# PREDICT-EPFL/piqp

Hardware: AMD Instinct MI355X
Metric: KKT factor+solve/sec (per IPM iter) (higher is better)
Workload: dtype f64; 1 GPU; dense QP n=4096 p=0 m_ineq=4096 (BASELINE configs[1]), kkt_solver=dense_cholesky, 1 update_scalings_and_factor + 2 KKTSystem::solve per step, inputs resident in HBM; n=4096, p=0, m=4096, parallelism=independent QP replicas x1

## Files before the change

piqp_amd/csrc/dense_kernels.hip:

```cpp
#include "dense_kernels.hpp"

#include <algorithm>
#include <map>
#include <mutex>
#include <stdexcept>
#include <utility>
#include <vector>
#include <cstdlib>
#include <cstdio>
#include <cstring>

namespace pq {
namespace dense {

typedef double d4 __attribute__((ext_vector_type(4)));
typedef double d2 __attribute__((ext_vector_type(2)));

__device__ __forceinline__ double readlane_d(double v, int srclane)
{
    long long bits = __double_as_longlong(v);
    int lo = (int)(bits & 0xffffffffll), hi = (int)(bits >> 32);
    lo = __builtin_amdgcn_readlane(lo, srclane);
    hi = __builtin_amdgcn_readlane(hi, srclane);
    return __longlong_as_double(((long long)hi << 32) | (unsigned int)lo);
}

template <bool FROM_LOWER>
__global__ __launch_bounds__(256) void k_symmetrize_upper(const double* __restrict__ Pu, int ldu, int n, double* __restrict__ Pf, double* __restrict__ pdiag)
{
    __shared__ double tile[32][33];
    const int r0 = blockIdx.x * 32, c0 = blockIdx.y * 32;
    const bool lower_tile = r0 > c0;
    const int sr0 = lower_tile ? c0 : r0, sc0 = lower_tile ? r0 : c0;
    const int tx = threadIdx.x & 31, ty = threadIdx.x >> 5;
    for (int cc = ty; cc < 32; cc += 8) {
        if constexpr (FROM_LOWER) {
            int c = sc0 + tx, r = sr0 + cc;
            tile[tx][cc] = (r < n && c < n) ? Pu[c + (size_t)r * ldu] : 0.0;
        } else {
            int r = sr0 + tx, c = sc0 + cc;
            tile[cc][tx] = (r < n && c < n) ? Pu[r + (size_t)c * ldu] : 0.0;
        }
    }
    __syncthreads();
    for (int cc = ty; cc < 32; cc += 8) {
        int i = r0 + tx, j = c0 + cc;
        if (i < n && j < n) {
            double v;
            if (lower_tile) v = tile[tx][cc];
            else if (r0 == c0) v = (tx <= cc) ? tile[cc][tx] : tile[tx][cc];
            else v = tile[cc][tx];
            Pf[i + (size_t)j * n] = v;
            if (i == j && pdiag) pdiag[i] = v;
        }
    }
}

#ifndef PQ_FUSE_TS
#define PQ_FUSE_TS 0
#endif
constexpr bool AGENT_OPERANDS = false;
constexpr bool FUSE_TS_ON = PQ_FUSE_TS != 0;
constexpr int TS = 128;
constexpr int BK = 16;
constexpr int LDS_LD = TS + 16;
constexpr int SYRK_LDS_BYTES = 2 * 2 * BK * LDS_LD * (int)sizeof(double);

__device__ __forceinline__ double ld_agent(const double* p);
__device__ __forceinline__ void st_agent(double* p, double v);
typedef __attribute__((address_space(1))) int gint;
__device__ __forceinline__ int ldi_agent(const int* p) { return __hip_atomic_load((const gint*)p, __ATOMIC_RELAXED, __HIP_MEMORY_SCOPE_AGENT); }
__device__ __forceinline__ void sti_agent(int* p, int v) { __hip_atomic_store((gint*)p, v, __ATOMIC_RELAXED, __HIP_MEMORY_SCOPE_AGENT); }
__device__ __forceinline__ int addi_agent(int* p, int v) { return __hip_atomic_fetch_add((gint*)p, v, __ATOMIC_RELAXED, __HIP_MEMORY_SCOPE_AGENT); }
template <bool CHECK, int NT>
__device__ __forceinline__ void load_tile(const double* __restrict__ M, int ld, int r0, int k0, int nrows, int kdim, int tid, d2 (&v)[1024 / NT])
{
    const int r = r0 + 2 * (tid & 63);
#pragma unroll
    for (int it = 0; it < 1024 / NT; ++it) {
        const int k = k0 + it * (NT / 64) + (tid >> 6);
        const __attribute__((address_space(1))) double* Mg = (const __attribute__((address_space(1))) double*)M;
        if (!CHECK) {
            v[it] = *reinterpret_cast<const __attribute__((address_space(1))) d2*>(Mg + r + (size_t)k * ld);
        } else {
            d2 t = {0.0, 0.0};
// ... 217 lines not shown
#pragma unroll
                    for (int q = 0; q < GRP; ++q) {
                        const int kt = g0 + q;
                        if (kt < nkt) {
                            const double* Asb = A4 + q * BK * LDS_LD + wr * SUBR + (lane & 15);
                            const double* Bsb = B4 + q * BK * LDS_LD + wc * SUBC + (lane & 15);
#pragma unroll
                            for (int ks = 0; ks < 4; ++ks) {
                                const int kk = ks * 4 + (lane >> 4);
                                double af[MTR], bf[MTC];
#pragma unroll
                                for (int u = 0; u < MTR; ++u) af[u] = Asb[kk * LDS_LD + u * 16];
#pragma unroll
                                for (int u = 0; u < MTC; ++u) bf[u] = Bsb[kk * LDS_LD + u * 16];
#pragma unroll
                                for (int x = 0; x < MTC; ++x)
#pragma unroll
                                    for (int y = 0; y < MTR; ++y)
                                        acc[x][y] = __builtin_amdgcn_mfma_f64_16x16x4f64(bf[x], af[y], acc[x][y], 0, 0, 0);
                            }
                        }
                    }
                }
            }
        }
        __syncthreads();
    }
    if (dbg_tile) a.fuse_ts[86] = clock64();
    if (tr_tile) a.fuse_tr2[42] = wall_clock64();
    if (tr_row) a.fuse_tr2[51] = wall_clock64();
    if constexpr (!QUARTER) {
        if (a.fuse_cnt && tj == 0 && a.fuse_pack) return panel_follow<NT, MTC, MTR, PERSIST, ROWS / 16>(a, smem, acc, row0, wr, wc, ti == 1);
    }
    if (skip_wave) return true;
#pragma unroll
    for (int x = 0; x < MTC; ++x) {
#pragma unroll
        for (int y = 0; y < MTR; ++y) {
            const int gi = row0 + wr * SUBR + y * 16 + (lane & 15);
#pragma unroll
            for (int r = 0; r < 4; ++r) {
                const int gj = col0 + wc * SUBC + x * 16 + (lane >> 4) + 4 * r;
                if (gi < a.n && gj < a.n && gi >= gj && gj < a.ncol) {
                    double* cp = a.C + (size_t)gi + (size_t)gj * a.ldc;
                    if (PERSIST) st_agent(cp, acc[x][y][r]);
                    else if constexpr (SUMSUB) *(__attribute__((address_space(1))) double*)cp = cfetch[x][y][r] - acc[x][y][r];
                    else *cp = acc[x][y][r];
                }
            }
        }
    }
    if (dbg_tile) { asm volatile("s_waitcnt vmcnt(0)" ::: "memory"); a.fuse_ts[87] = clock64(); }
    if (tr_tile) { a.fuse_tr2[43] = wall_clock64(); asm volatile("s_waitcnt vmcnt(0)" ::: "memory"); a.fuse_tr2[44] = wall_clock64(); }
    return true;
}

template <int EPI, int WR, int WC>
__device__ __forceinline__ void syrk_lower_body(const SyrkArgs& a, const int block_x)
{
    constexpr int NT = 64 * WR * WC;
    constexpr int MTR = 8 / WR, MTC = 8 / WC;
    constexpr int SUBR = TS / WR, SUBC = TS / WC;
    extern __shared__ __attribute__((aligned(16))) double smem[];
    double* As = smem;
    double* Bs = smem + 2 * BK * LDS_LD;

    int bid = block_x;
    if constexpr (EPI == EPI_SUBTRACT_POTRF) {
        if (bid < FUSE_ROLES) { fused_next_diag<NT, false>(a, smem, bid); return; }
        bid -= FUSE_ROLES - 1;
        const int T = (a.n + TS - 1) / TS;
        int ti, tj;
        if (bid <= T - 1) { ti = bid; tj = 0; }
        else {
            const int bb = bid - T;
            int t2 = (int)((sqrt(8.0 * (double)bb + 1.0) - 1.0) * 0.5);
            while ((t2 + 1) * (t2 + 2) / 2 <= bb) ++t2;
            while (t2 * (t2 + 1) / 2 > bb) --t2;
            ti = t2 + 1; tj = bb - t2 * (t2 + 1) / 2 + 1;
        }
        (void)fused_tile<NT, false>(a, ti, tj, smem);
        return;
    } else {
    const int b = a.tile_begin + bid / a.k_split;
    const int kslice = bid % a.k_split;
    int ti, tj;
    if (a.tile_order) {
        const int pk = a.tile_order[b];
        ti = pk >> 16; tj = pk & 0xffff;
    } else {
        ti = (int)((sqrt(8.0 * (double)b + 1.0) - 1.0) * 0.5);
        while ((ti + 1) * (ti + 2) / 2 <= b) ++ti;
        while (ti * (ti + 1) / 2 > b) --ti;
        tj = b - ti * (ti + 1) / 2;
    }
    const int row0 = ti * TS, col0 = tj * TS;
    if (col0 >= a.ncol) return;

    const int tid = threadIdx.x, lane = tid & 63, wave = tid >> 6;
    const int wr = wave / WC, wc = wave % WC;
    const bool edge = (row0 + TS > a.n) || (col0 + TS > a.n) || a.unaligned;
    const bool skip_wave = (ti == tj) && ((wr + 1) * SUBR <= wc * SUBC);

    d4 acc[MTC][MTR];
#pragma unroll
    for (int x = 0; x < MTC; ++x)
#pragma unroll
        for (int y = 0; y < MTR; ++y) acc[x][y] = (d4){0.0, 0.0, 0.0, 0.0};

    const int nkt_all = (a.kdim + BK - 1) / BK;
    const int kt_per = (nkt_all + a.k_split - 1) / a.k_split;
    const int kt_begin = kslice * kt_per;
    const int nkt = max(0, min(nkt_all, kt_begin + kt_per) - kt_begin);
    d2 va[1024 / NT], vb[1024 / NT];
    if (nkt > 0) {
        const int k0 = kt_begin * BK;
        const bool chk = edge || (k0 + BK > a.kdim);
        if (chk) { load_tile<true, NT>(a.A, a.lda, row0, k0, a.n, a.kdim, tid, va); load_tile<true, NT>(a.B, a.ldb, col0, k0, a.n, a.kdim, tid, vb); scale_tile<true, NT>(a.w, k0, a.kdim, tid, vb); }
        else { load_tile<false, NT>(a.A, a.lda, row0, k0, a.n, a.kdim, tid, va); load_tile<false, NT>(a.B, a.ldb, col0, k0, a.n, a.kdim, tid, vb); scale_tile<false, NT>(a.w, k0, a.kdim, tid, vb); }
        store_tile<NT>(As, tid, va);
        store_tile<NT>(Bs, tid, vb);
    }
    __syncthreads();

    for (int kt = 0; kt < nkt; ++kt) {
        const int cur = kt & 1;
        const bool more = (kt + 1 < nkt);
        if (more) {
            const int k0 = (kt_begin + kt + 1) * BK;
            const bool chk = edge || (k0 + BK > a.kdim);
            if (chk) { load_tile<true, NT>(a.A, a.lda, row0, k0, a.n, a.kdim, tid, va); load_tile<true, NT>(a.B, a.ldb, col0, k0, a.n, a.kdim, tid, vb); scale_tile<true, NT>(a.w, k0, a.kdim, tid, vb); }
            else { load_tile<false, NT>(a.A, a.lda, row0, k0, a.n, a.kdim, tid, va); load_tile<false, NT>(a.B, a.ldb, col0, k0, a.n, a.kdim, tid, vb); scale_tile<false, NT>(a.w, k0, a.kdim, tid, vb); }
        }
        if (!skip_wave) {
            const double* Asb = As + cur * BK * LDS_LD + wr * SUBR + (lane & 15);
            const double* Bsb = Bs + cur * BK * LDS_LD + wc * SUBC + (lane & 15);
#pragma unroll
            for (int ks = 0; ks < 4; ++ks) {
                const int kk = ks * 4 + (lane >> 4);
                double af[MTR], bf[MTC];
#pragma unroll
                for (int q = 0; q < MTR; ++q) af[q] = Asb[kk * LDS_LD + q * 16];
#pragma unroll
                for (int q = 0; q < MTC; ++q) bf[q] = Bsb[kk * LDS_LD + q * 16];
#pragma unroll
                for (int x = 0; x < MTC; ++x)
#pragma unroll
                    for (int y = 0; y < MTR; ++y)
                        acc[x][y] = __builtin_amdgcn_mfma_f64_16x16x4f64(bf[x], af[y], acc[x][y], 0, 0, 0);
            }
        }
        if (more) {
            store_tile<NT>(As + (cur ^ 1) * BK * LDS_LD, tid, va);
            store_tile<NT>(Bs + (cur ^ 1) * BK * LDS_LD, tid, vb);
        }
        __syncthreads();
    }

    if (skip_wave) return;
    if (a.part) {
        double* P = a.part + (size_t)block_x * TS * TS;
#pragma unroll
        for (int x = 0; x < MTC; ++x)
#pragma unroll
            for (int y = 0; y < MTR; ++y)
#pragma unroll
                for (int r = 0; r < 4; ++r)
                    P[(wr * SUBR + y * 16 + (lane & 15)) + (size_t)(wc * SUBC + x * 16 + (lane >> 4) + 4 * r) * TS] = acc[x][y][r];
        return;
    }
#pragma unroll
    for (int x = 0; x < MTC; ++x) {
#pragma unroll
        for (int y = 0; y < MTR; ++y) {
            const int gi = row0 + wr * SUBR + y * 16 + (lane & 15);
#pragma unroll
            for (int r = 0; r < 4; ++r) {
                const int gj = col0 + wc * SUBC + x * 16 + (lane >> 4) + 4 * r;
                if (gi < a.n && gj < a.n && gi >= gj && gj < a.ncol) {
                    const size_t ci = (size_t)gi + (size_t)gj * a.ldc;
                    const double v = acc[x][y][r];
                    if (EPI == EPI_ASSEMBLE) {
                        double base = a.Pfull[(size_t)gi + (size_t)gj * a.ldp];
                        if (gi == gj) base += a.x_reg[gi];
                        if (a.ATA) base += a.dinv * a.ATA[(size_t)gi + (size_t)gj * a.ldata];
                        ((__attribute__((address_space(1))) double*)a.C)[ci] = base + v;
                    } else if (EPI == EPI_SUBTRACT) {
                        ((__attribute__((address_space(1))) double*)a.C)[ci] -= v;
                    } else {
                        ((__attribute__((address_space(1))) double*)a.C)[ci] = v;
                    }
                }
            }
        }
    }
    }
}

template <int EPI, int WR, int WC>
__global__ __launch_bounds__(64 * WR * WC, (WR * WC == 4) ? 2 : (WR * WC == 8 ? 2 : 4)) void k_syrk_lower(SyrkArgs a)
{
    syrk_lower_body<EPI, WR, WC>(a, (int)blockIdx.x);
}

__device__ __forceinline__ bool front_panel(const FrontJob& j, int panel, int& k, int& nb, int& rs)
{
    k = panel * FACTOR_NB;
    if (k >= j.w) return false;
    nb = min(FACTOR_NB, j.w - k);
    rs = j.f - k - nb;
    return true;
}
template <int WR, int WC>
__global__ __launch_bounds__(64 * WR * WC, (WR * WC == 4) ? 2 : (WR * WC == 8 ? 2 : 4)) void k_syrk_lower_fronts(const FrontJob* __restrict__ jobs, int panel, int kind)
{
    const FrontJob j = jobs[blockIdx.y];
    if (kind >= 0 && j.kind != kind) return;
    int k, nb, rs;
    if (!front_panel(j, panel, k, nb, rs) || rs <= 0) return;
    const int T = (rs + TS - 1) / TS;
    if ((int)blockIdx.x >= T * (T + 1) / 2) return;
    SyrkArgs a;
    a.n = rs; a.kdim = nb;
    a.A = j.F + (k + nb) + (size_t)k * j.f; a.lda = j.f; a.B = a.A; a.ldb = j.f; a.w = j.dvec + k;
    a.C = j.F + (k + nb) + (size_t)(k + nb) * j.f; a.ldc = j.f;
    a.unaligned = ((j.f & 1) || (reinterpret_cast<uintptr_t>(a.A) & 15)) ? 1 : 0;
    if (j.multi) {
        a.ncol = j.w - (k + nb);
        if (a.ncol <= 0) return;
    }
    syrk_lower_body<EPI_SUBTRACT, WR, WC>(a, (int)blockIdx.x);
}
template <int WR, int WC>
__global__ __launch_bounds__(64 * WR * WC, (WR * WC == 4) ? 2 : (WR * WC == 8 ? 2 : 4)) void k_syrk_multi_fronts(const FrontJob* __restrict__ jobs)
{
    const FrontJob j = jobs[blockIdx.y];
    if (!j.multi || j.kind != 0) return;
    const int u = j.f - j.w;
    const int T = (u + TS - 1) / TS;
    if (u <= 0 || (int)blockIdx.x >= T * (T + 1) / 2) return;
    for (int k = 0; k < j.w; k += FACTOR_NB) {
        SyrkArgs a;
        a.n = u; a.kdim = min(FACTOR_NB, j.w - k);
        a.A = j.F + j.w + (size_t)k * j.f; a.lda = j.f; a.B = a.A; a.ldb = j.f; a.w = j.dvec + k;
        a.C = j.F + j.w + (size_t)j.w * j.f; a.ldc = j.f;
        a.unaligned = ((j.f & 1) || (reinterpret_cast<uintptr_t>(a.A) & 15)) ? 1 : 0;
        syrk_lower_body<EPI_SUBTRACT, WR, WC>(a, (int)blockIdx.x);
        __threadfence_block();
        __syncthreads();
    }
}

template <int SPLIT>
__global__ __launch_bounds__(512) void k_syrk_half_fronts(const FrontJob* __restrict__ jobs, int panel, int kind)
{
    const FrontJob j = jobs[blockIdx.y];
    if (kind >= 0 && j.kind != kind) return;
    int k, nb, rs;
    if (!front_panel(j, panel, k, nb, rs) || rs <= 0) return;
    const int T = (rs + TS - 1) / TS;
    const int b = (int)blockIdx.x / SPLIT, h = (int)blockIdx.x % SPLIT;
    if (b >= T * (T + 1) / 2) return;
    int ti = (int)((sqrt(8.0 * (double)b + 1.0) - 1.0) * 0.5);
    while ((ti + 1) * (ti + 2) / 2 <= b) ++ti;
    while (ti * (ti + 1) / 2 > b) --ti;
    const int tj = b - ti * (ti + 1) / 2;
    if (ti * TS + (TS / SPLIT) * h >= rs) return;
    SyrkArgs a;
    a.n = rs; a.kdim = nb;
    a.A = j.F + (k + nb) + (size_t)k * j.f; a.lda = j.f; a.B = a.A; a.ldb = j.f; a.w = j.dvec + k;
    a.C = j.F + (k + nb) + (size_t)(k + nb) * j.f; a.ldc = j.f;
    a.unaligned = ((j.f & 1) || (reinterpret_cast<uintptr_t>(a.A) & 15)) ? 1 : 0;
    if (j.multi) {
        a.ncol = j.w - (k + nb);
        if (a.ncol <= 0 || tj * TS >= a.ncol) return;
    }
    extern __shared__ __attribute__((aligned(16))) double smem[];
    (void)fused_tile<512, false, true, true, SPLIT == 4>(a, ti, tj, smem, h);
}

template <int EPI>
__global__ __launch_bounds__(256) void k_syrk_tail_reduce(SyrkArgs a)
{
    const int b = a.tile_begin + (int)blockIdx.x;
    int ti, tj;
    if (a.tile_order) {
        const int pk = a.tile_order[b];
        ti = pk >> 16; tj = pk & 0xffff;
    } else {
        ti = (int)((sqrt(8.0 * (double)b + 1.0) - 1.0) * 0.5);
        while ((ti + 1) * (ti + 2) / 2 <= b) ++ti;
        while (ti * (ti + 1) / 2 > b) --ti;
        tj = b - ti * (ti + 1) / 2;
    }
    const int row0 = ti * TS, col0 = tj * TS;
    const double* P0 = a.part + (size_t)blockIdx.x * a.k_split * TS * TS;
    {
        const int idx = (int)blockIdx.y * 256 + (int)threadIdx.x;
        const int li = idx & (TS - 1), lj = idx >> 7;
        const int gi = row0 + li, gj = col0 + lj;
        if (gi >= a.n || gj >= a.n || gi < gj) return;
        double v = 0.0;
#pragma unroll 8
        for (int sl = 0; sl < a.k_split; ++sl) v += P0[(size_t)sl * TS * TS + idx];
        const size_t ci = (size_t)gi + (size_t)gj * a.ldc;
        if (EPI == EPI_ASSEMBLE) {
            double base = a.Pfull[(size_t)gi + (size_t)gj * a.ldp];
            if (gi == gj) base += a.x_reg[gi];
            if (a.ATA) base += a.dinv * a.ATA[(size_t)gi + (size_t)gj * a.ldata];
            a.C[ci] = base + v;
        } else if (EPI == EPI_SUBTRACT) {
            a.C[ci] -= v;
        } else {
            a.C[ci] = v;
        }
    }
}

static int g_slots = 0;
static int syrk_slots()
{
    if (g_slots == 0) {
        int dev = 0, cus = 256;
        if (hipGetDevice(&dev) == hipSuccess) (void)hipDeviceGetAttribute(&cus, hipDeviceAttributeMultiprocessorCount, dev);
        g_slots = 2 * (cus > 0 ? cus : 256);
    }
    return g_slots;
}
static void syrk_tail_plan(int n, int kdim, int& rem, int& ksplit)
{
    const int T = div_up(n, TS);
    const int ntiles = T * (T + 1) / 2;
    const int slots = syrk_slots();
    const int nkt = div_up(kdim, BK);
    rem = ntiles % slots;
    ksplit = 1;
    if (ntiles > slots && rem > 0 && rem * 10 < slots * 6) {
        int s = slots / rem;
        s = std::min(s, nkt / 4);
        if (s >= 2) ksplit = s;
    }
    if (ksplit == 1) rem = 0;
}
size_t syrk_split_workspace_doubles(int n, int kdim)
{
    int rem, ks;
    syrk_tail_plan(n, kdim, rem, ks);
    return (size_t)rem * ks * TS * TS;
}

static const int* syrk_tile_order(int T)
{
    static std::mutex mu;
    static std::map<std::pair<int, int>, int*> cache;
    if (T < 16) return nullptr;
    int dev = 0;
    if (hipGetDevice(&dev) != hipSuccess) return nullptr;
    std::lock_guard<std::mutex> lk(mu);
    auto it = cache.find({dev, T});
    if (it != cache.end()) return it->second;
    constexpr int S = 8, NX = 8;
    std::vector<int> blocked;
    for (int SI = 0; SI * S < T; ++SI)
        for (int SJ = 0; SJ <= SI; ++SJ)
            for (int ti = SI * S; ti < std::min(T, SI * S + S); ++ti)
                for (int tj = SJ * S; tj < SJ * S + S && tj <= ti; ++tj) blocked.push_back(ti << 16 | tj);
    const int nt = (int)blocked.size();
    std::vector<int> start(NX + 1, 0);
    for (int x = 0; x < NX; ++x) start[x + 1] = start[x] + nt / NX + (x < nt % NX ? 1 : 0);
    std::vector<int> order(nt);
    for (int b = 0; b < nt; ++b) order[b] = blocked[start[b % NX] + b / NX];
    int* d = nullptr;
    if (hipMalloc(&d, sizeof(int) * nt) != hipSuccess) { (void)hipGetLastError(); cache[{dev, T}] = nullptr; return nullptr; }
    ++alloc_counter();
    if (hipMemcpy(d, order.data(), sizeof(int) * nt, hipMemcpyHostToDevice) != hipSuccess) { (void)hipGetLastError(); (void)hipFree(d); d = nullptr; }
    cache[{dev, T}] = d;
    return d;
}

void syrk_prepare(int n) { (void)syrk_tile_order(div_up(n, TS)); }

template <int EPI>
static void launch_syrk_t(SyrkArgs a, hipStream_t s, double* ws, size_t ws_doubles)
{
    const int T = div_up(a.n, TS);
    const int ntiles = T * (T + 1) / 2;
    int rem = 0, ks = 1;
    if (ws) syrk_tail_plan(a.n, a.kdim, rem, ks);
    if (rem > 0 && (size_t)rem * ks * TS * TS > ws_doubles) { rem = 0; ks = 1; }
    const int main_tiles = ntiles - rem;
    a.tile_begin = 0; a.k_split = 1; a.part = nullptr;
    const bool low_latency = a.kdim <= 256;
    a.tile_order = !low_latency ? syrk_tile_order(T) : nullptr;
    if (low_latency) hipLaunchKernelGGL((k_syrk_lower<EPI, 4, 4>), dim3(main_tiles), dim3(1024), SYRK_LDS_BYTES, s, a);
    else hipLaunchKernelGGL((k_syrk_lower<EPI, 2, 2>), dim3(main_tiles), dim3(256), SYRK_LDS_BYTES, s, a);
    if (rem > 0) {
        a.tile_begin = main_tiles; a.k_split = ks; a.part = ws;
        hipLaunchKernelGGL((k_syrk_lower<EPI, 2, 2>), dim3(rem * ks), dim3(256), SYRK_LDS_BYTES, s, a);
        hipLaunchKernelGGL(k_syrk_tail_reduce<EPI>, dim3(rem, TS * TS / 256), dim3(256), 0, s, a);
    }
}

void launch_syrk(int epi, const SyrkArgs& args_in, hipStream_t s, double* split_ws, size_t split_ws_doubles)
{
    SyrkArgs a = args_in;
    if (a.n <= 0) return;
    a.unaligned = ((a.lda & 1) || (a.ldb & 1) || (reinterpret_cast<uintptr_t>(a.A) & 15) || (reinterpret_cast<uintptr_t>(a.B) & 15)) ? 1 : 0;
    static PerDeviceOnce attr_set;
    attr_set([&] {
        PQ_HIP(hipFuncSetAttribute(reinterpret_cast<const void*>(k_syrk_lower<EPI_ASSEMBLE, 2, 2>), hipFuncAttributeMaxDynamicSharedMemorySize, SYRK_LDS_BYTES));
        PQ_HIP(hipFuncSetAttribute(reinterpret_cast<const void*>(k_syrk_lower<EPI_SUBTRACT, 2, 2>), hipFuncAttributeMaxDynamicSharedMemorySize, SYRK_LDS_BYTES));
        PQ_HIP(hipFuncSetAttribute(reinterpret_cast<const void*>(k_syrk_lower<EPI_STORE, 2, 2>), hipFuncAttributeMaxDynamicSharedMemorySize, SYRK_LDS_BYTES));
        PQ_HIP(hipFuncSetAttribute(reinterpret_cast<const void*>(k_syrk_lower<EPI_ASSEMBLE, 4, 4>), hipFuncAttributeMaxDynamicSharedMemorySize, SYRK_LDS_BYTES));
        PQ_HIP(hipFuncSetAttribute(reinterpret_cast<const void*>(k_syrk_lower<EPI_SUBTRACT, 4, 4>), hipFuncAttributeMaxDynamicSharedMemorySize, SYRK_LDS_BYTES));
        PQ_HIP(hipFuncSetAttribute(reinterpret_cast<const void*>(k_syrk_lower<EPI_STORE, 4, 4>), hipFuncAttributeMaxDynamicSharedMemorySize, SYRK_LDS_BYTES));
    });
    if (epi == EPI_SUBTRACT_POTRF) {
        static PerDeviceOnce fused_attr;
        fused_attr([&] {
            PQ_HIP(hipFuncSetAttribute(reinterpret_cast<const void*>(k_syrk_lower<EPI_SUBTRACT_POTRF, 4, 2>), hipFuncAttributeMaxDynamicSharedMemorySize, FUSED_LDS_BYTES));
        });
        const int T = div_up(a.n, TS);
        a.tile_begin = 0; a.k_split = 1; a.part = nullptr;
        if (!a.fuse_scratch || !a.fuse_flags || a.fuse_nb <= 0 || a.kdim > TS) throw std::runtime_error("fused trailing update: scratch / flags / panel width");
        hipLaunchKernelGGL((k_syrk_lower<EPI_SUBTRACT_POTRF, 4, 2>), dim3(T * (T + 1) / 2 + FUSE_ROLES - 1), dim3(512), FUSED_LDS_BYTES, s, a);
        PQ_HIP(hipGetLastError());
        return;
    }
    switch (epi) {
    case EPI_ASSEMBLE: launch_syrk_t<EPI_ASSEMBLE>(a, s, split_ws, split_ws_doubles); break;
    case EPI_SUBTRACT: launch_syrk_t<EPI_SUBTRACT>(a, s, split_ws, split_ws_doubles); break;
    default: launch_syrk_t<EPI_STORE>(a, s, split_ws, split_ws_doubles); break;
    }
    PQ_HIP(hipGetLastError());
}

__global__ __launch_bounds__(256) void k_assemble_no_g(int n, const double* __restrict__ Pf, const double* __restrict__ x_reg, const double* __restrict__ ATA, double dinv, double* __restrict__ C)
{
    const int j = blockIdx.y;
    const int i = blockIdx.x * 256 + threadIdx.x;
    if (i < n && i >= j) {
        double v = Pf[i + (size_t)j * n];
        if (i == j) v += x_reg[i];
        if (ATA) v += dinv * ATA[i + (size_t)j * n];
        C[i + (size_t)j * n] = v;
    }
}
void launch_assemble_no_g(int n, const double* Pf, const double* x_reg, const double* ATA, double dinv, double* C, hipStream_t s)
{
    if (n <= 0) return;
    hipLaunchKernelGGL(k_assemble_no_g, dim3(div_up(n, 256), n), dim3(256), 0, s, n, Pf, x_reg, ATA, dinv, C);
    PQ_HIP(hipGetLastError());
}


template <int NBLK, int LD, int NT = 256, bool TRANSPOSE = false>
__device__ __forceinline__ void stage_lower_block(const double* __restrict__ A, int lda, int nr, double* __restrict__ Ls, int tid)
{
    constexpr int PER_THREAD = NBLK * NBLK / NT;
    constexpr int BATCH = 16;
#pragma unroll 1
    for (int b0 = 0; b0 < PER_THREAD; b0 += BATCH) {
        double v[BATCH];
#pragma unroll
        for (int u = 0; u < BATCH; ++u) {
            const int idx = (b0 + u) * NT + tid;
            const int r = idx % NBLK, c = idx / NBLK;
            const bool ok = (r < nr) && (c < nr) && (r >= c);
            const double* p = ok ? (A + r + (size_t)c * lda) : A;
            const double t = *p;
            v[u] = ok ? t : ((r == c) ? 1.0 : 0.0);
        }
#pragma unroll
        for (int u = 0; u < BATCH; ++u) {
            const int idx = (b0 + u) * NT + tid;
            if (TRANSPOSE) Ls[(idx % NBLK) * LD + (idx / NBLK)] = v[u];
            else Ls[(idx / NBLK) * LD + (idx % NBLK)] = v[u];
        }
    }
}

__device__ __forceinline__ int tb_index(int bi, int bj) { return bi * (bi + 1) / 2 + bj; }
constexpr int TB_BLOCKS = 36;
constexpr int TB_DOUBLES = TB_BLOCKS * 256;
constexpr int POTRF_LDS_BYTES = (TB_DOUBLES + 8 * 32) * (int)sizeof(double);

__device__ __forceinline__ d4 tile_load(const double* __restrict__ blk, int lane)
{
    const double* p = blk + (lane >> 4) * 16 + (lane & 15);
    return (d4){p[0], p[64], p[128], p[192]};
}
__device__ __forceinline__ void tile_store(double* __restrict__ blk, int lane, d4 t)
{
    double* p = blk + (lane >> 4) * 16 + (lane & 15);
    p[0] = t[0]; p[64] = t[1]; p[128] = t[2]; p[192] = t[3];
}

__device__ __forceinline__ void wave_lds_sync()
{
    __builtin_amdgcn_fence(__ATOMIC_RELEASE, "wavefront");
    __builtin_amdgcn_wave_barrier();
    __builtin_amdgcn_fence(__ATOMIC_ACQUIRE, "wavefront");
}

constexpr int PIVOT_NEWTON = 2;
__device__ __forceinline__ double rsqrt_newton(double d)
// ... 2555 lines not shown
```

piqp_amd/csrc/dense_kernels.hpp:

```cpp
#pragma once

#include "common.hpp"

namespace pq {
namespace dense {

enum { EPI_ASSEMBLE = 0, EPI_SUBTRACT = 1, EPI_STORE = 2, EPI_SUBTRACT_POTRF = 3 };

struct SyrkArgs {
    int n = 0;
    int kdim = 0;
    const double* A = nullptr; int lda = 0;
    const double* B = nullptr; int ldb = 0;
    const double* w = nullptr;
    double* C = nullptr; int ldc = 0;
    const double* Pfull = nullptr; int ldp = 0;
    const double* x_reg = nullptr;
    const double* ATA = nullptr; int ldata = 0;
    double dinv = 0.0;
    int unaligned = 0;
    int ncol = 1 << 30;
    int tile_begin = 0;
    int k_split = 1;
    double* part = nullptr;
    int fuse_xwant = 0;
    const int* tile_order = nullptr;
    int fuse_nb = 0;
    int fuse_kglobal = 0;
    int fuse_ldlt = 0;
    int* fuse_info = nullptr;
    double* fuse_rdiag = nullptr;
    double* fuse_dvec = nullptr;
    double* fuse_pack = nullptr;
    int fuse_token = 0;
    int* fuse_flags = nullptr;
    double* fuse_scratch = nullptr;
    int* fuse_cnt = nullptr;
    double* fuse_w16 = nullptr;
    int* fuse_xpub = nullptr;
    const int* fuse_xcnt = nullptr;
    double* fuse_side = nullptr;
    long long* fuse_tr2 = nullptr;
    long long* fuse_tr2n = nullptr;
    int* fuse_abort = nullptr;
    const int* late_p[2] = {nullptr, nullptr};
    int late_w[2] = {0, 0};
    long long* fuse_ts = nullptr;
};

void launch_syrk(int epi, const SyrkArgs& args, hipStream_t s, double* split_ws = nullptr, size_t split_ws_doubles = 0);
size_t syrk_split_workspace_doubles(int n, int kdim);
void syrk_prepare(int n);
void launch_assemble_no_g(int n, const double* Pf, const double* x_reg, const double* ATA, double dinv, double* C, hipStream_t s);
void launch_potrf_diag(bool ldlt, double* A, int lda, int nb, int kglobal, int* info, double* rdiag, double* dvec, double* pack, double* w16, hipStream_t s,
                       long long* ts = nullptr);
double microbench_potrf_block(bool ldlt, int reps, long long* stamps64, hipStream_t s);
int debug_potrf_block(bool ldlt, int nb, int reps, const double* A_host, double* L_host, double* rdiag_host, double* dvec_host, double* pack_host, int* info_host, hipStream_t s);
void launch_trsm_panel(bool ldlt, double* A, int lda, int k0, int nb, int n, const double* pack, const double* rdiag, hipStream_t s);
bool chol_persistent_supported(int n);
bool chol_prepare(int n);
size_t chol_flag_ints(int n);
int chol_debug_plan(int T, int* out5, int capacity_tasks);
bool launch_chol_persistent(bool ldlt, double* A, double* side, int lda, int n, int* info, double* rdiag, double* dvec, double* pack2, double* w16, double* scratch, int* fuse_flags, int* fuse_cnt,
                            int token_base, int* flags, int gen, int fcount, hipStream_t s);
size_t trsv_poll_doubles(int n);
void launch_trsv_poll_init(double* ypoll, int n, hipStream_t s);
void launch_trsv(const double* L, int ld, int n, double* x, const double* rdiag, bool ldlt, double* ypoll, int* ctl, const double* w16, hipStream_t s, long long* ts = nullptr,
                 const double* Vinv = nullptr, int xcd_seq = -1);
bool probe_one_xcd_sweeps(hipStream_t s);
void launch_block_inverse_dd(bool unit, const double* L, int ld, int n, double* Vsq, hipStream_t s);
size_t block_inverse_dd_doubles(int n);
int gemv_n_slices(int rows, int cols);
int launch_gemv_n_partial(int rows, int cols, const double* M, int ld, const double* v, const double* scale, double alpha, double* part, hipStream_t s);
void launch_reduce_partials(int rows, int nslices, const double* part, const double* base, double* y, hipStream_t s);
void launch_gemv_t(int rows, int cols, const double* M, int ld, const double* v, double alpha, double beta, const double* c, const double* sc, double* out, hipStream_t s);
void launch_symmetrize_upper(const double* Pu, int n, double* Pf, double* pdiag, hipStream_t s);
void launch_symmetrize(const double* A, int lda, bool from_lower, int n, double* Pf, double* pdiag, hipStream_t s);
void launch_reciprocal(int n, const double* a, double* out, hipStream_t s);
void launch_flag_nonpositive(int n, const double* rdiag, int* info, hipStream_t s);
double microbench_mfma_f64(int iters, hipStream_t s);
double microbench_hbm_copy(size_t bytes, int iters, hipStream_t s);

constexpr int FACTOR_NB = 128;
constexpr int FACTOR_PACK_DOUBLES = 36 * 256;

struct FrontJob {
    double* F = nullptr;
    int f = 0, w = 0, first = 0;
    double* pack = nullptr;
    double* dvec = nullptr;
    int kind = 0;
    int multi = 0;
    int* cnt = nullptr;
};
constexpr int FRONT_CNT_PANELS = 16, FRONT_CNT_INTS = 160;
void launch_front_diag_panels(const FrontJob* jobs_device, int njobs, int panel, int max_rows_below, int* info, double* rdiag, hipStream_t s, bool follow = false);
void launch_front_updates(const FrontJob* jobs_device, int njobs, int panel, int max_rows_below, hipStream_t s, int kind = -1);
void launch_front_updates_multi(const FrontJob* jobs_device, int njobs, int max_update_rows, hipStream_t s);
bool launch_front_panel_step(const FrontJob* jobs_device, int njobs, int panel, int max_rows_below, int* info, double* rdiag, hipStream_t s);

}
}
```

piqp_amd/csrc/dense_kkt.cpp:

```cpp
#include <algorithm>
#include <cstdio>
#include <cstdlib>
#include <stdexcept>
#include <string>
#include <vector>

#include "trace.hpp"
#include "dense_kernels.hpp"
#include "kkt_solver_base.hpp"

namespace pq {

namespace {

class DenseKKT final : public KKTSolverBase {
public:
    DenseKKT(const pq_dense_data* d, int kkt_solver, int device) : dev_(device), n_(d->n), p_(d->p), m_(d->m), ldlt_(kkt_solver == PQ_DENSE_LDLT_NO_PIVOT)
    {
        if (n_ <= 0 || p_ < 0 || m_ < 0) throw std::runtime_error("dense KKT: bad dimensions");
        PQ_HIP(hipSetDevice(dev_));
        PQ_HIP(hipStreamCreateWithFlags(&st_, hipStreamNonBlocking));
        alloc();
        upload(d);
    }
// ... 85 lines not shown
    void eval_G_xn_and_GT_xt(double alpha_n, double alpha_t, const double* xn, const double* xt, double* zn, double* zt) override
    {
        PQ_HIP(hipSetDevice(dev_));
        if (m_ > 0) dense::launch_gemv_t(n_, m_, GT_.p, n_, xn, alpha_n, 0.0, nullptr, nullptr, zn, st_);
        int nsl = 0;
        if (m_ > 0) nsl = dense::launch_gemv_n_partial(n_, m_, GT_.p, n_, xt, nullptr, alpha_t, part_.p, st_);
        dense::launch_reduce_partials(n_, nsl, part_.p, nullptr, zt, st_);
    }

    void print_info() override {}

    const double* P_diag_device() const override { return Pdiag_.p; }
    int n() const override { return n_; }
    int p() const override { return p_; }
    int m() const override { return m_; }
    hipStream_t stream() const override { return st_; }
    int device() const override { return dev_; }

    void internal_kkt_mat(double* out_host) override
    {
        PQ_HIP(hipSetDevice(dev_));
        DBuf<double> tmp((size_t)n_ * n_);
        tmp.zero(st_);
        update_kkt(x_reg_last_.p, tmp.p);
        PQ_HIP(hipMemcpyAsync(out_host, tmp.p, sizeof(double) * (size_t)n_ * n_, hipMemcpyDeviceToHost, st_));
        stream_wait(st_);
    }
    void set_profiling(int level) override { prof_.enabled = level != 0; prof_.level = level; }
    void get_profile(int stage, double* total_ms, int* count) override
    {
        if (stage < 0 || stage >= StageProfiler::NSTAGE) throw std::runtime_error("bad stage");
        PQ_HIP(hipSetDevice(dev_));
        prof_.collect(stage, st_, total_ms, count);
    }
    void set_class_failure_semantics(bool on) override { class_semantics_ = on; }
    bool factor_symmetric(const double* A_dev, int lda, bool from_lower) override
    {
        if (p_ != 0 || m_ != 0) throw std::runtime_error("factor_symmetric: a handle with p = m = 0 only");
        PQ_HIP(hipSetDevice(dev_));
        join_inverses();
        delta_ = 1.0;
        dense::launch_symmetrize(A_dev, lda, from_lower, n_, fac_.p, nullptr, st_);
        const int t1 = prof_.begin(1, st_);
        launch_factor_panels();
        prof_.end(1, t1, st_);
        if (inv_sweeps_) {
            PQ_HIP(hipEventRecord(ev_fac_, st_));
            PQ_HIP(hipStreamWaitEvent(st_inv_, ev_fac_, 0));
            dense::launch_block_inverse_dd(ldlt_, fac_.p, n_, n_, vinv_.p, st_inv_);
            PQ_HIP(hipEventRecord(ev_inv_, st_inv_));
            inv_pending_ = true;
        }
        return factor_status();
    }
    void internal_factor(double* out_host) override
    {
        PQ_HIP(hipSetDevice(dev_));
        PQ_HIP(hipMemcpyAsync(out_host, fac_.p, sizeof(double) * (size_t)n_ * n_, hipMemcpyDeviceToHost, st_));
        stream_wait(st_);
    }

private:
    DenseKKT(const DenseKKT& o, int) : dev_(o.dev_), n_(o.n_), p_(o.p_), m_(o.m_), ldlt_(o.ldlt_), class_semantics_(o.class_semantics_), delta_(o.delta_)
    {
        PQ_HIP(hipStreamCreateWithFlags(&st_, hipStreamNonBlocking));
        alloc();
        auto cp = [&](DBuf<double>& dst, const DBuf<double>& src) { if (src.n) PQ_HIP(hipMemcpyAsync(dst.p, src.p, src.bytes(), hipMemcpyDeviceToDevice, st_)); };
        cp(Pfull_, o.Pfull_); cp(Pdiag_, o.Pdiag_); cp(AT_, o.AT_); cp(GT_, o.GT_); cp(ATA_, o.ATA_); cp(fac_, o.fac_);
        cp(vinv_, o.vinv_);
        cp(z_reg_inv_, o.z_reg_inv_); cp(x_reg_last_, o.x_reg_last_); cp(rdiag_, o.rdiag_); cp(w16_, o.w16_);
        stream_wait(st_);
    }

    void alloc()
    {
        const size_t nn = (size_t)n_ * n_;
        Pfull_.alloc(nn); Pdiag_.alloc(n_);
        AT_.alloc((size_t)n_ * p_); GT_.alloc((size_t)n_ * m_);
        if (p_ > 0) ATA_.alloc(nn);
        fac_.alloc(nn);
        z_reg_inv_.alloc(m_); x_reg_last_.alloc(n_); dvec_.alloc(n_); rdiag_.alloc(n_);
        const int sl = dense::gemv_n_slices(n_, m_ > 0 ? m_ : 1) + dense::gemv_n_slices(n_, p_ > 0 ? p_ : 1) + dense::gemv_n_slices(n_, n_);
        part_.alloc((size_t)sl * n_);
        split_ws_.alloc(dense::syrk_split_workspace_doubles(n_, m_ > 0 ? m_ : 1));
        pack_.alloc(dense::FACTOR_PACK_DOUBLES);
        fuse_scratch_.alloc(dense::FACTOR_PACK_DOUBLES); fuse_flags_.alloc(16); fuse_flags_.zero(st_); fuse_cnt_.alloc(8); fuse_cnt_.zero(st_);
        w16_.alloc((size_t)((n_ + 127) / 128) * 8 * 256);
        dense::syrk_prepare(n_);
        info_.alloc(1);
        info_h_.alloc(2);
        info_h_.p[0] = -1; info_h_.p[1] = 0;
        chol_persistent_ = !debug_token("chol_launches") && dense::chol_prepare(n_);
        if (chol_persistent_) { side_.alloc((size_t)n_ * n_); pack2_.alloc(2 * (size_t)dense::FACTOR_PACK_DOUBLES); chol_flags_.alloc(dense::chol_flag_ints(n_)); chol_flags_.zero(st_); }
        flags_.alloc(3); flags_.zero(st_);
        one_xcd_ = (n_ + 127) / 128 <= 32 && !debug_token("no_one_xcd") && dense::probe_one_xcd_sweeps(st_);
        ypoll_.alloc(dense::trsv_poll_doubles(n_)); dense::launch_trsv_poll_init(ypoll_.p, n_, st_);
        inv_sweeps_ = (n_ + 127) / 128 >= 8 && (n_ + 127) / 128 <= 224;
        if (const char* e = debug_token("inv_sweeps")) inv_sweeps_ = std::atoi(e) != 0 && (n_ + 127) / 128 <= 224;
        if (inv_sweeps_) {
            vinv_.alloc(dense::block_inverse_dd_doubles(n_));
            PQ_HIP(hipStreamCreateWithFlags(&st_inv_, hipStreamNonBlocking));
            PQ_HIP(hipEventCreateWithFlags(&ev_fac_, hipEventDisableTiming));
            PQ_HIP(hipEventCreateWithFlags(&ev_inv_, hipEventDisableTiming));
        }
        if (debug_token("trsv_ts")) { trsv_ts_.alloc(4 * ((n_ + 127) / 128) + 8); trsv_ts_.zero(st_); }
        if (const char* e = debug_token("fused_ts")) { dbg_panel_ = std::atoi(e); dbg_ts_.alloc(96); dbg_ts_.zero(st_); }
        x_reg_last_.zero(st_);
        fac_.zero(st_);
    }

    void upload(const pq_dense_data* d)
    {
        const size_t nn = (size_t)n_ * n_;
        copy_in(fac_.p, d->P_utri, nn * sizeof(double), d->mem, st_);
        dense::launch_symmetrize_upper(fac_.p, n_, Pfull_.p, Pdiag_.p, st_);
        copy_in(AT_.p, d->AT, (size_t)n_ * p_ * sizeof(double), d->mem, st_);
        copy_in(GT_.p, d->GT, (size_t)n_ * m_ * sizeof(double), d->mem, st_);
        if (p_ > 0) {
            dense::SyrkArgs a;
            a.n = n_; a.kdim = p_; a.A = AT_.p; a.lda = n_; a.B = AT_.p; a.ldb = n_; a.C = ATA_.p; a.ldc = n_;
            dense::launch_syrk(dense::EPI_STORE, a, st_);
        }
        stream_wait(st_);
    }

    void update_kkt(const double* x_reg, double* out)
    {
        const double dinv = 1.0 / delta_;
        if (m_ > 0) {
            dense::launch_syrk(dense::EPI_ASSEMBLE, assembly_args(x_reg, out), st_, split_ws_.p, split_ws_.n);
        } else {
            dense::launch_assemble_no_g(n_, Pfull_.p, x_reg, p_ > 0 ? ATA_.p : nullptr, dinv, out, st_);
        }
    }

    dense::SyrkArgs assembly_args(const double* x_reg, double* out) const
    {
        dense::SyrkArgs a;
        a.n = n_; a.kdim = m_; a.A = GT_.p; a.lda = n_; a.B = GT_.p; a.ldb = n_; a.w = z_reg_inv_.p; a.C = out; a.ldc = n_;
        a.Pfull = Pfull_.p; a.ldp = n_; a.x_reg = x_reg; a.ATA = p_ > 0 ? ATA_.p : nullptr; a.ldata = n_; a.dinv = 1.0 / delta_;
        return a;
    }

    void launch_factor_panels()
    {
        PQ_HIP(hipMemsetAsync(info_.p, 0xFF, sizeof(int), st_));
        const int NB = dense::FACTOR_NB;
        if (chol_persistent_) {
            dense::launch_potrf_diag(ldlt_, fac_.p, n_, NB, 0, info_.p, rdiag_.p, dvec_.p, pack_.p, w16_.p, st_);
            { const int tt = prof_.begin(4, st_); dense::launch_trsm_panel(ldlt_, fac_.p, n_, 0, NB, n_, pack_.p, rdiag_.p, st_); prof_.end(4, tt, st_); }
            const int T = n_ / NB;
            if (chol_gen_ > 0x3fffffff - 2 * (T + 2)) { chol_flags_.zero(st_); chol_gen_ = 0; chol_fcount_ = 0; }
            chol_gen_ += T + 2;
            const int tt = prof_.begin(3, st_);
            if (!dense::launch_chol_persistent(ldlt_, fac_.p, side_.p, n_, n_, info_.p, rdiag_.p, dvec_.p, pack2_.p, w16_.p, fuse_scratch_.p, fuse_flags_.p, fuse_cnt_.p, fuse_token_, chol_flags_.p,
                                               chol_gen_, chol_fcount_, st_))
                throw std::runtime_error("dense factorisation: the persistent launch has no plan for this size / device");
            prof_.end(3, tt, st_);
            fuse_token_ += T - 1;
            ++chol_fcount_;
            return;
        }
        int p = 0;
        for (int k = 0; k < n_; k += NB, ++p) {
            const int nb = (n_ - k < NB) ? n_ - k : NB;
            const int rs = n_ - k - nb;
            double* A11 = fac_.p + k + (size_t)k * n_;
// ... 112 lines not shown
```

Baseline: 347.7 IPM-iter KKT (1 factor + 2 solves)/s.

## Replace tail k-split SYRK with stream-K balanced persistent kernel for assembly

Replaces the main SYRK launch plus separate k-split tail launch and reduction kernel with a single persistent stream-K style kernel for the KKT assembly SYRK. Each workgroup receives an equal share of (tile, k-block) iterations within its XCD. Workgroups that finish a partial tile publish it to a workspace with a token flag, and the tile's head workgroup spins on that flag before adding the partial in its epilogue. This targets wave-quantization imbalance and removes extra launches. In exchange it adds inter-workgroup spin-waiting, a timeout that writes NaN poison, and a dependence on all slots being co-resident.

After: 338.7 IPM-iter KKT (1 factor + 2 solves)/s (median of 2 runs). Within noise of the previous version (-2.6%).

```diff
diff --git a/piqp_amd/csrc/dense_kernels.hip b/piqp_amd/csrc/dense_kernels.hip
--- a/piqp_amd/csrc/dense_kernels.hip
+++ b/piqp_amd/csrc/dense_kernels.hip
@@ -1,6 +1,7 @@
 #include "dense_kernels.hpp"
 
 #include <algorithm>
+#include <atomic>
 #include <map>
 #include <mutex>
 #include <stdexcept>
@@ -384,8 +385,7 @@
         (void)fused_tile<NT, false>(a, ti, tj, smem);
         return;
     } else {
-    const int b = a.tile_begin + bid / a.k_split;
-    const int kslice = bid % a.k_split;
+    const int b = bid;
     int ti, tj;
     if (a.tile_order) {
         const int pk = a.tile_order[b];
@@ -410,13 +410,10 @@
 #pragma unroll
         for (int y = 0; y < MTR; ++y) acc[x][y] = (d4){0.0, 0.0, 0.0, 0.0};
 
-    const int nkt_all = (a.kdim + BK - 1) / BK;
-    const int kt_per = (nkt_all + a.k_split - 1) / a.k_split;
-    const int kt_begin = kslice * kt_per;
-    const int nkt = max(0, min(nkt_all, kt_begin + kt_per) - kt_begin);
+    const int nkt = (a.kdim + BK - 1) / BK;
     d2 va[1024 / NT], vb[1024 / NT];
     if (nkt > 0) {
-        const int k0 = kt_begin * BK;
+        const int k0 = 0;
         const bool chk = edge || (k0 + BK > a.kdim);
         if (chk) { load_tile<true, NT>(a.A, a.lda, row0, k0, a.n, a.kdim, tid, va); load_tile<true, NT>(a.B, a.ldb, col0, k0, a.n, a.kdim, tid, vb); scale_tile<true, NT>(a.w, k0, a.kdim, tid, vb); }
         else { load_tile<false, NT>(a.A, a.lda, row0, k0, a.n, a.kdim, tid, va); load_tile<false, NT>(a.B, a.ldb, col0, k0, a.n, a.kdim, tid, vb); scale_tile<false, NT>(a.w, k0, a.kdim, tid, vb); }
@@ -429,7 +426,7 @@
         const int cur = kt & 1;
         const bool more = (kt + 1 < nkt);
         if (more) {
-            const int k0 = (kt_begin + kt + 1) * BK;
+            const int k0 = (kt + 1) * BK;
             const bool chk = edge || (k0 + BK > a.kdim);
             if (chk) { load_tile<true, NT>(a.A, a.lda, row0, k0, a.n, a.kdim, tid, va); load_tile<true, NT>(a.B, a.ldb, col0, k0, a.n, a.kdim, tid, vb); scale_tile<true, NT>(a.w, k0, a.kdim, tid, vb); }
             else { load_tile<false, NT>(a.A, a.lda, row0, k0, a.n, a.kdim, tid, va); load_tile<false, NT>(a.B, a.ldb, col0, k0, a.n, a.kdim, tid, vb); scale_tile<false, NT>(a.w, k0, a.kdim, tid, vb); }
@@ -460,17 +457,6 @@
     }
 
     if (skip_wave) return;
-    if (a.part) {
-        double* P = a.part + (size_t)block_x * TS * TS;
-#pragma unroll
-        for (int x = 0; x < MTC; ++x)
-#pragma unroll
-            for (int y = 0; y < MTR; ++y)
-#pragma unroll
-                for (int r = 0; r < 4; ++r)
-                    P[(wr * SUBR + y * 16 + (lane & 15)) + (size_t)(wc * SUBC + x * 16 + (lane >> 4) + 4 * r) * TS] = acc[x][y][r];
-        return;
-    }
 #pragma unroll
     for (int x = 0; x < MTC; ++x) {
 #pragma unroll
@@ -582,39 +568,149 @@
 }
 
 template <int EPI>
-__global__ __launch_bounds__(256) void k_syrk_tail_reduce(SyrkArgs a)
-{
-    const int b = a.tile_begin + (int)blockIdx.x;
-    int ti, tj;
-    if (a.tile_order) {
-        const int pk = a.tile_order[b];
-        ti = pk >> 16; tj = pk & 0xffff;
-    } else {
-        ti = (int)((sqrt(8.0 * (double)b + 1.0) - 1.0) * 0.5);
-        while ((ti + 1) * (ti + 2) / 2 <= b) ++ti;
-        while (ti * (ti + 1) / 2 > b) --ti;
-        tj = b - ti * (ti + 1) / 2;
-    }
-    const int row0 = ti * TS, col0 = tj * TS;
-    const double* P0 = a.part + (size_t)blockIdx.x * a.k_split * TS * TS;
-    {
-        const int idx = (int)blockIdx.y * 256 + (int)threadIdx.x;
-        const int li = idx & (TS - 1), lj = idx >> 7;
-        const int gi = row0 + li, gj = col0 + lj;
-        if (gi >= a.n || gj >= a.n || gi < gj) return;
-        double v = 0.0;
-#pragma unroll 8
-        for (int sl = 0; sl < a.k_split; ++sl) v += P0[(size_t)sl * TS * TS + idx];
-        const size_t ci = (size_t)gi + (size_t)gj * a.ldc;
-        if (EPI == EPI_ASSEMBLE) {
-            double base = a.Pfull[(size_t)gi + (size_t)gj * a.ldp];
-            if (gi == gj) base += a.x_reg[gi];
-            if (a.ATA) base += a.dinv * a.ATA[(size_t)gi + (size_t)gj * a.ldata];
-            a.C[ci] = base + v;
-        } else if (EPI == EPI_SUBTRACT) {
-            a.C[ci] -= v;
+__device__ __forceinline__ void syrk_store_tile(const SyrkArgs& a, const d4 (&acc)[4][4], int row0, int col0, int wr, int wc, int lane, const double* __restrict__ tail, bool poison)
+{
+#pragma unroll
+    for (int x = 0; x < 4; ++x) {
+#pragma unroll
+        for (int y = 0; y < 4; ++y) {
+            const int li = wr * 64 + y * 16 + (lane & 15);
+            const int gi = row0 + li;
+#pragma unroll
+            for (int r = 0; r < 4; ++r) {
+                const int lj = wc * 64 + x * 16 + (lane >> 4) + 4 * r;
+                const int gj = col0 + lj;
+                if (tail) asm volatile("" ::: "memory");
+                if (gi < a.n && gj < a.n && gi >= gj) {
+                    const size_t ci = (size_t)gi + (size_t)gj * a.ldc;
+                    double v = acc[x][y][r];
+                    if (tail) v += ld_agent(tail + li + lj * TS);
+                    if (poison) v = __builtin_nan("");
+                    if (EPI == EPI_ASSEMBLE) {
+                        double base = a.Pfull[(size_t)gi + (size_t)gj * a.ldp];
+                        if (gi == gj) base += a.x_reg[gi];
+                        if (a.ATA) base += a.dinv * a.ATA[(size_t)gi + (size_t)gj * a.ldata];
+                        ((__attribute__((address_space(1))) double*)a.C)[ci] = base + v;
+                    } else {
+                        ((__attribute__((address_space(1))) double*)a.C)[ci] = v;
+                    }
+                }
+            }
+        }
+    }
+}
+
+template <int EPI>
+__global__ __launch_bounds__(256, 2) void k_syrk_balanced(SyrkArgs a)
+{
+    constexpr int NT = 256, WC = 2, SUB = 64;
+    extern __shared__ __attribute__((aligned(16))) double smem[];
+    __shared__ int ok_s;
+    double* As = smem;
+    double* Bs = smem + 2 * BK * LDS_LD;
+    const int tid = threadIdx.x, lane = tid & 63, wave = tid >> 6;
+    const int wr = wave / WC, wc = wave % WC;
+    const int g = (int)blockIdx.x, J = (int)gridDim.x >> 3, xcd = g & 7;
+    const int T = (a.n + TS - 1) / TS, ntiles = T * (T + 1) / 2, nkt = (a.kdim + BK - 1) / BK;
+    const int cnt = ntiles / 8 + (xcd < ntiles % 8 ? 1 : 0);
+    const long long total = (long long)cnt * nkt;
+    const int run = J - 1 - (g >> 3);
+    const int s_begin = (int)(run * total / J), s_end = (int)((run + 1) * total / J);
+    int* const abort_w = a.sk_flags + gridDim.x;
+
+    for (int s = s_begin; s < s_end;) {
+        const int it = s / nkt, kb = s - it * nkt, ke = min(nkt, kb + (s_end - s));
+        s += ke - kb;
+        const int pk = a.tile_order[xcd + 8 * it];
+        const int ti = pk >> 16, tj = pk & 0xffff;
+        const int row0 = ti * TS, col0 = tj * TS;
+        const bool edge = (row0 + TS > a.n) || (col0 + TS > a.n) || a.unaligned;
+        const bool skip_wave = (ti == tj) && ((wr + 1) * SUB <= wc * SUB);
+
+        d4 acc[4][4];
+#pragma unroll
+        for (int x = 0; x < 4; ++x)
+#pragma unroll
+            for (int y = 0; y < 4; ++y) acc[x][y] = (d4){0.0, 0.0, 0.0, 0.0};
+
+        d2 va[1024 / NT], vb[1024 / NT];
+        {
+            const int k0 = kb * BK;
+            const bool chk = edge || (k0 + BK > a.kdim);
+            if (chk) { load_tile<true, NT>(a.A, a.lda, row0, k0, a.n, a.kdim, tid, va); load_tile<true, NT>(a.B, a.ldb, col0, k0, a.n, a.kdim, tid, vb); scale_tile<true, NT>(a.w, k0, a.kdim, tid, vb); }
+            else { load_tile<false, NT>(a.A, a.lda, row0, k0, a.n, a.kdim, tid, va); load_tile<false, NT>(a.B, a.ldb, col0, k0, a.n, a.kdim, tid, vb); scale_tile<false, NT>(a.w, k0, a.kdim, tid, vb); }
+            store_tile<NT>(As, tid, va);
+            store_tile<NT>(Bs, tid, vb);
+        }
+        __syncthreads();
+        for (int kt = kb; kt < ke; ++kt) {
+            const int cur = (kt - kb) & 1;
+            const bool more = (kt + 1 < ke);
+            if (more) {
+                const int k0 = (kt + 1) * BK;
+                const bool chk = edge || (k0 + BK > a.kdim);
+                if (chk) { load_tile<true, NT>(a.A, a.lda, row0, k0, a.n, a.kdim, tid, va); load_tile<true, NT>(a.B, a.ldb, col0, k0, a.n, a.kdim, tid, vb); scale_tile<true, NT>(a.w, k0, a.kdim, tid, vb); }
+                else { load_tile<false, NT>(a.A, a.lda, row0, k0, a.n, a.kdim, tid, va); load_tile<false, NT>(a.B, a.ldb, col0, k0, a.n, a.kdim, tid, vb); scale_tile<false, NT>(a.w, k0, a.kdim, tid, vb); }
+            }
+            if (!skip_wave) {
+                const double* Asb = As + cur * BK * LDS_LD + wr * SUB + (lane & 15);
+                const double* Bsb = Bs + cur * BK * LDS_LD + wc * SUB + (lane & 15);
+#pragma unroll
+                for (int ks = 0; ks < 4; ++ks) {
+                    const int kk = ks * 4 + (lane >> 4);
+                    double af[4], bf[4];
+#pragma unroll
+                    for (int q = 0; q < 4; ++q) af[q] = Asb[kk * LDS_LD + q * 16];
+#pragma unroll
+                    for (int q = 0; q < 4; ++q) bf[q] = Bsb[kk * LDS_LD + q * 16];
+#pragma unroll
+                    for (int x = 0; x < 4; ++x)
+#pragma unroll
+                        for (int y = 0; y < 4; ++y)
+                            acc[x][y] = __builtin_amdgcn_mfma_f64_16x16x4f64(bf[x], af[y], acc[x][y], 0, 0, 0);
+                }
+            }
+            if (more) {
+                store_tile<NT>(As + (cur ^ 1) * BK * LDS_LD, tid, va);
+                store_tile<NT>(Bs + (cur ^ 1) * BK * LDS_LD, tid, vb);
+            }
+            __syncthreads();
+        }
+
+        int lane_e = lane;
+        asm volatile("" : "+v"(lane_e));
+        if (kb > 0) {
+            if (!skip_wave) {
+                double* P = a.part + (size_t)g * TS * TS + (wr * SUB + (lane_e & 15)) + (wc * SUB + (lane_e >> 4)) * TS;
+#pragma unroll
+                for (int x = 0; x < 4; ++x)
+#pragma unroll
+                    for (int y = 0; y < 4; ++y) {
+#pragma unroll
+                        for (int r = 0; r < 4; ++r) st_agent(P + y * 16 + (x * 16 + 4 * r) * TS, acc[x][y][r]);
+                        asm volatile("" ::: "memory");
+                    }
+            }
+            __threadfence();
+            __syncthreads();
+            if (tid == 0) sti_agent(a.sk_flags + g, a.sk_token);
         } else {
-            a.C[ci] = v;
+            const bool head = ke < nkt;
+            if (head && tid == 0) {
+                int ok = 1;
+                unsigned spins = 0;
+                while (ldi_agent(a.sk_flags + g - 8) != a.sk_token) {
+                    __builtin_amdgcn_s_sleep(8);
+                    ++spins;
+                    if ((spins & 255u) == 0 && ldi_agent(abort_w) == a.sk_token) { ok = 0; break; }
+                    if (spins > 8000000u) { ok = 0; sti_agent(abort_w, a.sk_token); break; }
+                }
+                ok_s = ok;
+            }
+            if (head) __syncthreads();
+            const bool ok = !head || ok_s != 0;
+            if (!skip_wave) syrk_store_tile<EPI>(a, acc, row0, col0, wr, wc, lane_e, head ? a.part + (size_t)(g - 8) * TS * TS : nullptr, !ok);
+            if (head) __syncthreads();
         }
     }
 }
@@ -629,26 +725,17 @@
     }
     return g_slots;
 }
-static void syrk_tail_plan(int n, int kdim, int& rem, int& ksplit)
+static bool syrk_balanced_fits(int n, int kdim)
 {
     const int T = div_up(n, TS);
-    const int ntiles = T * (T + 1) / 2;
     const int slots = syrk_slots();
-    const int nkt = div_up(kdim, BK);
-    rem = ntiles % slots;
-    ksplit = 1;
-    if (ntiles > slots && rem > 0 && rem * 10 < slots * 6) {
-        int s = slots / rem;
-        s = std::min(s, nkt / 4);
-        if (s >= 2) ksplit = s;
-    }
-    if (ksplit == 1) rem = 0;
+    return kdim > 256 && T >= 16 && slots % 8 == 0 && (T * (T + 1) / 2) / 8 >= slots / 8;
 }
 size_t syrk_split_workspace_doubles(int n, int kdim)
 {
-    int rem, ks;
-    syrk_tail_plan(n, kdim, rem, ks);
-    return (size_t)rem * ks * TS * TS;
+    if (!syrk_balanced_fits(n, kdim)) return 0;
+    const size_t slots = (size_t)syrk_slots();
+    return slots * TS * TS + (slots + 2) / 2;
 }
 
 static const int* syrk_tile_order(int T)
@@ -687,20 +774,22 @@
 {
     const int T = div_up(a.n, TS);
     const int ntiles = T * (T + 1) / 2;
-    int rem = 0, ks = 1;
-    if (ws) syrk_tail_plan(a.n, a.kdim, rem, ks);
-    if (rem > 0 && (size_t)rem * ks * TS * TS > ws_doubles) { rem = 0; ks = 1; }
-    const int main_tiles = ntiles - rem;
-    a.tile_begin = 0; a.k_split = 1; a.part = nullptr;
+    a.part = nullptr;
     const bool low_latency = a.kdim <= 256;
     a.tile_order = !low_latency ? syrk_tile_order(T) : nullptr;
-    if (low_latency) hipLaunchKernelGGL((k_syrk_lower<EPI, 4, 4>), dim3(main_tiles), dim3(1024), SYRK_LDS_BYTES, s, a);
-    else hipLaunchKernelGGL((k_syrk_lower<EPI, 2, 2>), dim3(main_tiles), dim3(256), SYRK_LDS_BYTES, s, a);
-    if (rem > 0) {
-        a.tile_begin = main_tiles; a.k_split = ks; a.part = ws;
-        hipLaunchKernelGGL((k_syrk_lower<EPI, 2, 2>), dim3(rem * ks), dim3(256), SYRK_LDS_BYTES, s, a);
-        hipLaunchKernelGGL(k_syrk_tail_reduce<EPI>, dim3(rem, TS * TS / 256), dim3(256), 0, s, a);
-    }
+    if constexpr (EPI == EPI_ASSEMBLE) {
+        if (ws && a.tile_order && a.ncol >= a.n && syrk_balanced_fits(a.n, a.kdim) && ws_doubles >= syrk_split_workspace_doubles(a.n, a.kdim)) {
+            static std::atomic<unsigned> token{0};
+            const int slots = syrk_slots();
+            unsigned t = ++token;
+            if ((t & 0x7fffffffu) == 0) t = ++token;
+            a.part = ws; a.sk_flags = reinterpret_cast<int*>(ws + (size_t)slots * TS * TS); a.sk_token = (int)(t & 0x7fffffffu);
+            hipLaunchKernelGGL(k_syrk_balanced<EPI>, dim3(slots), dim3(256), SYRK_LDS_BYTES, s, a);
+            return;
+        }
+    }
+    if (low_latency) hipLaunchKernelGGL((k_syrk_lower<EPI, 4, 4>), dim3(ntiles), dim3(1024), SYRK_LDS_BYTES, s, a);
+    else hipLaunchKernelGGL((k_syrk_lower<EPI, 2, 2>), dim3(ntiles), dim3(256), SYRK_LDS_BYTES, s, a);
 }
 
 void launch_syrk(int epi, const SyrkArgs& args_in, hipStream_t s, double* split_ws, size_t split_ws_doubles)
@@ -716,6 +805,7 @@
         PQ_HIP(hipFuncSetAttribute(reinterpret_cast<const void*>(k_syrk_lower<EPI_ASSEMBLE, 4, 4>), hipFuncAttributeMaxDynamicSharedMemorySize, SYRK_LDS_BYTES));
         PQ_HIP(hipFuncSetAttribute(reinterpret_cast<const void*>(k_syrk_lower<EPI_SUBTRACT, 4, 4>), hipFuncAttributeMaxDynamicSharedMemorySize, SYRK_LDS_BYTES));
         PQ_HIP(hipFuncSetAttribute(reinterpret_cast<const void*>(k_syrk_lower<EPI_STORE, 4, 4>), hipFuncAttributeMaxDynamicSharedMemorySize, SYRK_LDS_BYTES));
+        PQ_HIP(hipFuncSetAttribute(reinterpret_cast<const void*>(k_syrk_balanced<EPI_ASSEMBLE>), hipFuncAttributeMaxDynamicSharedMemorySize, SYRK_LDS_BYTES));
     });
     if (epi == EPI_SUBTRACT_POTRF) {
         static PerDeviceOnce fused_attr;
@@ -723,7 +813,7 @@
             PQ_HIP(hipFuncSetAttribute(reinterpret_cast<const void*>(k_syrk_lower<EPI_SUBTRACT_POTRF, 4, 2>), hipFuncAttributeMaxDynamicSharedMemorySize, FUSED_LDS_BYTES));
         });
         const int T = div_up(a.n, TS);
-        a.tile_begin = 0; a.k_split = 1; a.part = nullptr;
+        a.part = nullptr;
         if (!a.fuse_scratch || !a.fuse_flags || a.fuse_nb <= 0 || a.kdim > TS) throw std::runtime_error("fused trailing update: scratch / flags / panel width");
         hipLaunchKernelGGL((k_syrk_lower<EPI_SUBTRACT_POTRF, 4, 2>), dim3(T * (T + 1) / 2 + FUSE_ROLES - 1), dim3(512), FUSED_LDS_BYTES, s, a);
         PQ_HIP(hipGetLastError());
diff --git a/piqp_amd/csrc/dense_kernels.hpp b/piqp_amd/csrc/dense_kernels.hpp
--- a/piqp_amd/csrc/dense_kernels.hpp
+++ b/piqp_amd/csrc/dense_kernels.hpp
@@ -20,9 +20,9 @@
     double dinv = 0.0;
     int unaligned = 0;
     int ncol = 1 << 30;
-    int tile_begin = 0;
-    int k_split = 1;
     double* part = nullptr;
+    int* sk_flags = nullptr;
+    int sk_token = 0;
     int fuse_xwant = 0;
     const int* tile_order = nullptr;
     int fuse_nb = 0;
diff --git a/piqp_amd/csrc/dense_kkt.cpp b/piqp_amd/csrc/dense_kkt.cpp
--- a/piqp_amd/csrc/dense_kkt.cpp
+++ b/piqp_amd/csrc/dense_kkt.cpp
@@ -191,7 +191,7 @@
         z_reg_inv_.alloc(m_); x_reg_last_.alloc(n_); dvec_.alloc(n_); rdiag_.alloc(n_);
         const int sl = dense::gemv_n_slices(n_, m_ > 0 ? m_ : 1) + dense::gemv_n_slices(n_, p_ > 0 ? p_ : 1) + dense::gemv_n_slices(n_, n_);
         part_.alloc((size_t)sl * n_);
-        split_ws_.alloc(dense::syrk_split_workspace_doubles(n_, m_ > 0 ? m_ : 1));
+        split_ws_.alloc(dense::syrk_split_workspace_doubles(n_, m_ > 0 ? m_ : 1)); split_ws_.zero(st_);
         pack_.alloc(dense::FACTOR_PACK_DOUBLES);
         fuse_scratch_.alloc(dense::FACTOR_PACK_DOUBLES); fuse_flags_.alloc(16); fuse_flags_.zero(st_); fuse_cnt_.alloc(8); fuse_cnt_.zero(st_);
         w16_.alloc((size_t)((n_ + 127) / 128) * 8 * 256);
```
